# chorowski-lab/pytorch-asr

Measured on AMD Instinct MI355X. Metric: CTC train-step frames/sec, higher is better.
Workload: dtype bf16; 1 GPU; WSJ mono-char CTC (egs/wsj/yamls/ctc.yaml shapes), DeepSpeech2 conv+4xBiLSTM-320 encoder + FSTDecoder, fwd+bwd+GradientClipping(clip 480000, skip 4.8e+06 = recipe x global_batch/16)+PolyakDecay+Adam, synthetic 40-dim x 1-channel x 1000-frame fbank; batch_per_gpu=768, global_batch=768, frames=1000, classes=49, parallelism=dp1, batch_norm=per-replica statistics, optimizer_steps=139, step_boundary=device: att_speech.fused_step (clip / skip decision + Adam, no read-back)

## Files before the change

include/asr_amd.h:

```cpp
#ifndef ASR_AMD_H
#define ASR_AMD_H

#include <stdint.h>

#ifdef __cplusplus
extern "C" {
#endif

enum {
    ASR_OK = 0,
    ASR_EINVAL = 1,
    ASR_EUNSUPPORTED = 2,
    ASR_ELAUNCH = 3
};

int asr_abi_version(void);

const char *asr_strerror(int code);

int64_t asr_lattice_fwbw_workspace_bytes(int T, int B, int C, int N);

int asr_lattice_fwbw_f32(const float *lp, int T, int B, int C,
                         const int32_t *lens,
                         const int32_t *src_in, const int32_t *il_in,
// ... 169 lines not shown
int64_t asr_conv7x7c32_workspace_bytes(void);
int asr_conv7x7c32_fwd_bf16(const void *x, const float *w, int B, int H, int W, int stride_h,
                            void *y, double *chan_sums, void *workspace, int64_t workspace_bytes,
                            void *stream);
int asr_conv7x7c32_bwd_data_bf16(const void *dy, const float *w, int B, int H, int W,
                                 int stride_h, void *dx, void *workspace,
                                 int64_t workspace_bytes, void *stream);
int asr_conv7x7c32_wgrad_bf16(const void *x, const void *dy, int B, int H, int W, int stride_h,
                              float *dw, void *workspace, int64_t workspace_bytes, void *stream);

int64_t asr_conv1_7x7s2_workspace_bytes(void);
int asr_conv1_7x7s2_fwd(const float *x, const float *w, int B, int T, int F, void *y,
                        double *chan_sums, void *workspace, int64_t workspace_bytes, void *stream);
int asr_conv1_7x7s2_wgrad(const float *x, const void *dy, int B, int T, int F, float *dw,
                          void *workspace, int64_t workspace_bytes, void *stream);

int64_t asr_conv1c_7x7s2_workspace_bytes(int cin);
int asr_conv1c_7x7s2_fwd(const float *x, const float *w, int B, int T, int F, int cin, void *y,
                         double *chan_sums, void *workspace, int64_t workspace_bytes, void *stream);
int asr_conv1c_7x7s2_wgrad(const float *x, const void *dy, int B, int T, int F, int cin,
                           float *dw, void *workspace, int64_t workspace_bytes, void *stream);

int asr_tcn_attention_step_f32(const float *eproj, const float *enc, const int32_t *enc_lens,
                               const float *filt, const float *glob, const float *w_score,
                               float b_score, float temperature,
                               const float *att_prev, const int32_t *parent,
                               int T, int B, int beam, int A, int Kf, int E,
                               float *att_new, float *context, void *stream);

int asr_tcn_attention_scan_fwd_f32(const float *eproj, const float *filt, const float *glob,
// ... 123 lines not shown
```

pytorch-asr_amd/att_speech/_native.py:

```python
import ctypes
import warnings
import os

import torch

_HERE = os.path.dirname(os.path.abspath(__file__))
LIB_PATH = os.environ.get(
    'ASR_AMD_LIB', os.path.join(os.path.dirname(_HERE), 'csrc', 'libasr_amd.so'))

ASR_OK, ASR_EINVAL, ASR_EUNSUPPORTED, ASR_ELAUNCH = 0, 1, 2, 3
ABI_VERSION = 24

_lib = None
EVENT_HOOK = None
_WARNED = {}

_vp, _i, _i64, _f = ctypes.c_void_p, ctypes.c_int, ctypes.c_int64, ctypes.c_float

_SIGNATURES = {
    'asr_abi_version': (ctypes.c_int, []),
    'asr_strerror': (ctypes.c_char_p, [_i]),
    'asr_lattice_fwbw_workspace_bytes': (_i64, [_i, _i, _i, _i]),
    'asr_lattice_fwbw_f32': (_i, [_vp, _i, _i, _i, _vp, _vp, _vp, _vp, _vp, _vp,
                                  _vp, _vp, _i, _i, _i, _i, _f, _vp, _vp, _vp,
# ... 9 lines not shown
    'asr_lattice_viterbi_workspace_bytes': (_i64, [_i, _i, _i]),
    'asr_lattice_forward_f32': (_i, [_vp, _i, _i, _i, _vp, _vp, _vp, _vp, _vp,
                                     _i, _i, _i, _f, _i, _vp, _vp, _vp, _i64,
                                     _vp]),
    'asr_log_softmax_fwd_f32': (_i, [_vp, _i64, _i, _vp, _vp]),
    'asr_log_softmax_bwd_f32': (_i, [_vp, _vp, _i64, _i, _vp, _vp]),
    'asr_sub_rowmax_f32': (_i, [_vp, _i, _i, _i, _vp, _vp, _vp, _vp, _vp]),
    'asr_argmax_rows_f32': (_i, [_vp, _i64, _i, _vp, _vp]),
    'asr_conv7x7c32_workspace_bytes': (_i64, []),
    'asr_conv7x7c32_fwd_bf16': (_i, [_vp, _vp, _i, _i, _i, _i, _vp, _vp, _vp, _i64, _vp]),
    'asr_conv7x7c32_bwd_data_bf16': (_i, [_vp, _vp, _i, _i, _i, _i, _vp, _vp, _i64, _vp]),
    'asr_conv7x7c32_wgrad_bf16': (_i, [_vp, _vp, _i, _i, _i, _i, _vp, _vp, _i64, _vp]),
    'asr_conv1_7x7s2_workspace_bytes': (_i64, []),
    'asr_conv1_7x7s2_fwd': (_i, [_vp, _vp, _i, _i, _i, _vp, _vp, _vp, _i64, _vp]),
    'asr_conv1_7x7s2_wgrad': (_i, [_vp, _vp, _i, _i, _i, _vp, _vp, _i64, _vp]),
    'asr_conv1c_7x7s2_workspace_bytes': (_i64, [_i]),
    'asr_conv1c_7x7s2_fwd': (_i, [_vp, _vp, _i, _i, _i, _i, _vp, _vp, _vp, _i64, _vp]),
    'asr_conv1c_7x7s2_wgrad': (_i, [_vp, _vp, _i, _i, _i, _i, _vp, _vp, _i64, _vp]),
    'asr_log_softmax_shift_fwd_f32': (_i, [_vp, _i, _i, _i, _vp, _vp, _vp, _vp, _vp]),
    'asr_log_softmax_shift_bwd_f32': (_i, [_vp, _vp, _vp, _i64, _i, _vp, _vp]),
    'asr_sum_leading_f32': (_i, [_vp, _i, _i64, _vp, _vp]),
    'asr_adam_chunk_elems': (_i, []),
    'asr_grad_sumsq_partials_f32': (_i, [_vp, _i64, _vp, _i, _vp]),
    'asr_adam_clip_step_f32': (_i, [_vp, _i, _vp, _vp, _vp, _vp, _i, _vp, _f, _f, _f, _f, _f, _f, _f,
                                    _vp, _vp, _vp, _vp]),
    'asr_adam_clip_step_ex_f32': (_i, [_vp, _i, _vp, _vp, _vp, _vp, _i, _vp, _f, _f, _f, _f, _f, _f, _f,
                                       _vp, _vp, _vp, _vp, _vp]),
    'asr_nonfinite_flag_f32': (_i, [_vp, _i, _vp, _vp]),
    'asr_noise_chunk_elems': (_i, []),
    'asr_gaussian_noise_f32': (_i, [_vp, _i, ctypes.c_uint64, ctypes.c_uint32, ctypes.c_uint64, _i, _i, _vp]),
# ... 1120 lines not shown
    if cin == 1:
        nbytes = L.asr_conv1_7x7s2_workspace_bytes()
        ws = torch.empty(nbytes, dtype=torch.uint8, device=x.device)
        check(L.asr_conv1_7x7s2_wgrad(_p(x), _p(dy), B, T, F, _p(dw), _p(ws), nbytes, _stream()),
              'asr_conv1_7x7s2_wgrad')
    else:
        nbytes = L.asr_conv1c_7x7s2_workspace_bytes(cin)
        if nbytes < 0:
            raise NotImplementedError('conv1_wgrad: %d input channels' % cin)
        ws = torch.empty(nbytes, dtype=torch.uint8, device=x.device)
        check(L.asr_conv1c_7x7s2_wgrad(_p(x), _p(dy), B, T, F, cin, _p(dw), _p(ws), nbytes, _stream()),
              'asr_conv1c_7x7s2_wgrad')
    return dw


def split_bf16(x, hi=None, lo=None):
    x = _dev(x, torch.float32, 'x')
    if hi is None:
        hi = torch.empty(x.shape, dtype=torch.bfloat16, device=x.device)
        lo = torch.empty(x.shape, dtype=torch.bfloat16, device=x.device)
        rows, cols, ldx, ldh, ldl = 1, x.numel(), x.numel(), x.numel(), x.numel()
    else:
        if x.dim() != 2 or hi.shape != x.shape or lo.shape != x.shape or x.stride(1) != 1 \
                or hi.stride(1) != 1 or lo.stride(1) != 1 or hi.dtype != torch.bfloat16 or lo.dtype != torch.bfloat16:
            raise ValueError('split_bf16: x, hi, lo must be [rows, cols] with a dense last dimension')
        rows, cols = x.shape
        ldx, ldh, ldl = x.stride(0), hi.stride(0), lo.stride(0)
    check(lib().asr_split_bf16_f32(_p(x), rows, cols, ldx, _p(hi), ldh, _p(lo), ldl, _stream()),
          'asr_split_bf16_f32')
    return hi, lo
# ... 65 lines not shown
```

pytorch-asr_amd/att_speech/modules/encoders/deep_speech_2.py:

```python
import warnings
from collections import OrderedDict

import torch
from torch import nn

from att_speech.modules.encoders.base_encoder import BaseEncoder
from att_speech.modules.encoders.encoder_utils import (
    BatchRNN, Normalization, SequentialWithOptionalAttributes)


class DeepSpeech2(BaseEncoder):
    def __init__(self, sample_batch, conv_normalization='batch_norm',
                 conv_strides=[[2, 2], [2, 1]],
                 conv_kernel_sizes=[[41, 11], [21, 11]],
                 conv_num_features=[32, 32],
                 rnn_hidden_size=768, rnn_nb_layers=5, rnn_projection_size=0,
                 rnn_type=nn.LSTM, rnn_dropout=0.0, rnn_residual=False,
                 rnn_normalization='batch_norm', rnn_subsample=None, **kwargs):
        super(DeepSpeech2, self).__init__(**kwargs)
        import os
        self.conv_bf16 = os.environ.get('ASR_CONV_BF16', '1') != '0'
        self.fused_bn = os.environ.get('ASR_FUSED_BN', '1') != '0'
        self.native_conv = os.environ.get('ASR_NATIVE_CONV', '1') != '0'
        if isinstance(rnn_type, str):
            rnn_type = {'LSTM': nn.LSTM, 'GRU': nn.GRU}[rnn_type.split('.')[-1]]
        self.makeConv(sample_batch, conv_strides, conv_kernel_sizes,
                      conv_num_features, conv_normalization)
        features = sample_batch['features']
        features = features.permute(0, 3, 1, 2)
        with torch.no_grad():
            was_training = self.conv.training
            self.conv.eval()
            after_conv_size = self.conv.forward(features).size()
            self.conv.train(was_training)
        self.rnn_input_size = after_conv_size[1] * after_conv_size[3]
        self.makeRnn(rnn_hidden_size, rnn_nb_layers, rnn_projection_size,
                     rnn_type, rnn_dropout, rnn_residual, rnn_normalization,
                     rnn_subsample)
# ... 62 lines not shown
                                            c.dilation, c.groups)
            y = nn.functional.conv2d(
                x.to(torch.bfloat16), c.weight.to(torch.bfloat16),
                None if bias is None else bias.to(torch.bfloat16),
                c.stride, c.padding, c.dilation, c.groups)
            return y if keep_bf16 else y.float()

        def second_conv(x, with_bias=True):
            return run_conv(c2, x, with_bias)

        if fused:
            from att_speech.modules.encoders.native_bn import bn_hardtanh
            from att_speech.modules.encoders import native_conv
            c1 = conv[0]
            sums1 = sums2 = None
            if bf16 and self.native_conv and native_conv.first_supported(c1, features):
                x, sums1 = native_conv.conv1(features, c1)
            else:
                if bf16 and self.native_conv and not getattr(self, '_warned_conv1', False):
                    self._warned_conv1 = True
                    warnings.warn('DeepSpeech2: the first convolution is not a (1 or 3)->32 7x7 stride-(1,2) '
                                  'shape on gradient-free features csrc/conv.hip is built for; using '
                                  'torch / MIOpen for it')
                x = run_conv(c1, features, with_bias=False, keep_bf16=True)
            x = bn_hardtanh(x, conv[1].batch_norm, conv[2], out_bf16=bf16, conv_bias=c1.bias,
                            chan_sums=sums1)
            if bf16 and self.native_conv and native_conv.supported(c2, x):
                y2, sums2 = native_conv.conv7x7c32(x, c2)
            else:
                if bf16 and self.native_conv and not getattr(self, '_warned_conv', False):
                    self._warned_conv = True
                    warnings.warn('DeepSpeech2: the second convolution is not the 32->32 7x7 '
                                  'stride-(3,1) shape csrc/conv.hip is built for; using torch / MIOpen')
                y2 = run_conv(c2, x, with_bias=False, keep_bf16=True)
            x = bn_hardtanh(y2, conv[4].batch_norm, conv[5], time_major=True, conv_bias=c2.bias,
                            chan_sums=sums2, out_bf16=bf16 and self._rnn_takes_bf16(y2))
            return x.view(x.size(0), x.size(1), -1)
        if bf16:
            x = conv[5](conv[4](second_conv(conv[2](conv[1](conv[0](features))))))
        else:
            x = conv(features)
# ... 24 lines not shown
```

pytorch-asr_amd/att_speech/modules/encoders/native_bn.py:

```python
import torch
import torch.distributed as dist

from att_speech import _native

SYNC = {'on': False, 'group': None}


def _sync_active():
    return (SYNC['on'] and dist.is_available() and dist.is_initialized()
            and dist.get_world_size(SYNC['group']) > 1)


def _allreduce_sums(sums, n_local):
    buf = torch.cat([sums.reshape(-1), sums.new_tensor([n_local])])
    dist.all_reduce(buf, op=dist.ReduceOp.SUM, group=SYNC['group'])
    sums.copy_(buf[:-1].view_as(sums))
    return float(buf[-1])


class BNHardtanhFunction(torch.autograd.Function):
    @staticmethod
    def forward(ctx, x, gamma, beta, conv_bias, running_mean, running_var, training, momentum,
                eps, lo, hi, out_bf16, time_major, chan_sums=None, sync_counts=None):
        out, mean, invstd = _native.bn_act_fwd(
# ... 10 lines not shown
        ctx.cfg = (training, lo, hi, time_major)
        ctx.sync = training and _sync_active()
        return out

    @staticmethod
    def backward(ctx, dy):
        x, gamma, beta, mean, invstd, cb = ctx.saved_tensors
        training, lo, hi, time_major = ctx.cfg
        dx, dgamma, dbeta, dcb = _native.bn_act_bwd(
            x, gamma.detach(), beta.detach(), mean, invstd, training, lo, hi, dy,
            time_major=time_major, conv_bias=cb.detach() if ctx.has_cb else None,
            sync=_allreduce_sums if ctx.sync else None)
        return (dx, dgamma, dbeta, dcb) + (None,) * 11


def bn_hardtanh(x, bn, act, out_bf16=False, time_major=False, conv_bias=None, chan_sums=None):
    use_batch_stats = bn.training or bn.running_mean is None
    momentum = 0.0
    rm = rv = None
    if use_batch_stats and bn.training and bn.track_running_stats and bn.running_mean is not None:
        bn.num_batches_tracked.add_(1)
        momentum = bn.momentum if bn.momentum is not None else 1.0 / float(bn.num_batches_tracked)
        rm, rv = bn.running_mean, bn.running_var
    elif not use_batch_stats:
        rm, rv = bn.running_mean, bn.running_var
    if x.dtype != torch.bfloat16:
        x = x.float()
    sync_counts = None
    if use_batch_stats and bn.training and _sync_active():
        n_local = float(x.shape[0] * x.shape[2] * x.shape[3])
        if chan_sums is None:
            xd = x.double()
            chan_sums = torch.stack([xd.sum((0, 2, 3)), (xd * xd).sum((0, 2, 3))])
        else:
            chan_sums = chan_sums.clone()
        n_total = _allreduce_sums(chan_sums, n_local)
        chan_sums.mul_(n_local / n_total)
        sync_counts = (n_local, n_total)
    return BNHardtanhFunction.apply(x, bn.weight, bn.bias, conv_bias, rm, rv, use_batch_stats,
                                    momentum, bn.eps, float(act.min_val), float(act.max_val),
# ... 3 lines not shown
```

pytorch-asr_amd/att_speech/modules/encoders/native_conv.py:

```python
import torch

from att_speech import _native


def supported(conv, x):
    return (x.is_cuda and isinstance(conv, torch.nn.Conv2d) and conv.in_channels == 32
            and conv.out_channels == 32 and tuple(conv.kernel_size) == (7, 7)
            and tuple(conv.stride) == (3, 1) and tuple(conv.padding) == (0, 0)
            and tuple(conv.dilation) == (1, 1) and conv.groups == 1
            and x.dim() == 4 and x.size(2) >= 7 and 7 <= x.size(3) <= 48)


class Conv7x7C32Function(torch.autograd.Function):
    @staticmethod
    def forward(ctx, x, weight):
        x = x.to(torch.bfloat16).contiguous(memory_format=torch.channels_last)
        ctx.save_for_backward(x, weight)
        y, sums = _native.conv7x7c32_fwd(x, weight.detach(), 3, want_sums=True)
        ctx.mark_non_differentiable(sums)
        return y, sums

    @staticmethod
    def backward(ctx, dy, _dsums):
        x, weight = ctx.saved_tensors
# ... 25 lines not shown
        ctx.mark_non_differentiable(sums)
        return y, sums

    @staticmethod
    def backward(ctx, dy, _dsums):
        x, weight = ctx.saved_tensors
        return None, (_native.conv1_wgrad(x, dy) if ctx.needs_input_grad[1] else None)


def conv1(features, conv):
    if features.size(1) == 1:
        return Conv1Function.apply(features[:, 0], conv.weight)
    return Conv1Function.apply(features.permute(0, 2, 3, 1), conv.weight)


def conv7x7c32(x, conv):
    return Conv7x7C32Function.apply(x, conv.weight)
```

pytorch-asr_amd/csrc/bnact.hip:

```cpp
#include "common.h"
#include "../../include/asr_amd.h"

namespace {

using namespace asr;

struct BnParams {
    const float *x;
    int B, C, HW, Wd;
    const float *gamma, *beta;
    const float *mean, *invstd;
    const float *shift;
    float lo, hi;
};

__global__ __launch_bounds__(256) void bn_stats_kernel(const float *x, const float *shift, int C, int HW, double *sums) {
    __shared__ float red[64];
    const int c = blockIdx.x, b = blockIdx.y;
    const float *p = x + ((size_t)b * C + c) * HW;
    const float sh0 = shift ? shift[c] : 0.f;
    float s = 0.f, q = 0.f;
    for (int i = threadIdx.x; i < HW; i += 256) {
        const float v = p[i] + sh0;
        s += v;
// ... 529 lines not shown

__global__ void zero_doubles_kernel(double *p, int n) {
    const int i = blockIdx.x * blockDim.x + threadIdx.x;
    if (i < n) p[i] = 0.0;
}

inline int tm_rows(int cw) {
    if (cw <= 0) return 0;
    const int fit = 48 * 1024 / (cw * 4);
    return fit < 8 ? fit : 8;
}

inline bool bad_shape(int B, int C, int H, int W) {
    return B <= 0 || C <= 0 || H <= 0 || W <= 0 || C > 65535 || B > 65535 ||
           (int64_t)H * W > 0x7fffffff;
}

}

extern "C" int64_t asr_bn_act_workspace_bytes(int C) { return C < 0 ? -1 : (int64_t)C * 2 * 8 + 64; }

extern "C" int asr_bn_act_fwd_f32(const void *x, int x_bf16, const float *conv_bias, int B, int C, int H, int W,
                                  const float *gamma, const float *beta,
                                  float *running_mean, float *running_var,
                                  int channels_last,
                                  int training, float momentum, float eps, float lo, float hi,
                                  void *out, int out_bf16, int out_time_major,
                                  float *save_mean, float *save_invstd,
                                  const double *chan_sums,
                                  void *workspace, int64_t workspace_bytes, void *stream) {
// ... 195 lines not shown
```

pytorch-asr_amd/csrc/conv.hip:

```cpp
#include <type_traits>
#include "common.h"
#include "../../include/asr_amd.h"

namespace {

typedef __attribute__((ext_vector_type(8))) __bf16 bf16x8;
typedef __attribute__((ext_vector_type(16))) float f32x16;
typedef __attribute__((ext_vector_type(4))) unsigned int u32x4;
typedef __attribute__((ext_vector_type(4))) float f32x4;
typedef __attribute__((ext_vector_type(4))) __bf16 bf16x4;

constexpr int CH = 32;
constexpr int KS = 7;
constexpr int PIX = 80;
constexpr int KSTEPS = KS * KS * CH / 16;

typedef __attribute__((ext_vector_type(4))) int rsrc_words;
__device__ __forceinline__ rsrc_words conv_raw_rsrc(const void *base, unsigned bytes) {
    const unsigned long long a = (unsigned long long)base;
    rsrc_words r;
    r.x = __builtin_amdgcn_readfirstlane((int)(unsigned)a);
    r.y = __builtin_amdgcn_readfirstlane((int)((unsigned)(a >> 32) & 0xffffu));
    r.z = __builtin_amdgcn_readfirstlane((int)bytes);
    r.w = 0x00020000;
    return r;
// ... 671 lines not shown
        const int t = t0 - 6 + (int)row;
        bf16x8 v = {};
        if (t >= 0 && t < p.T) {
            const float2 *src = reinterpret_cast<const float2 *>(xb + (size_t)t * p.F + 2 * fo);
#pragma unroll
            for (int j = 0; j < 4; ++j) {
                const float2 f2 = src[j];
                v[2 * j] = (__bf16)f2.x;
                v[2 * j + 1] = (__bf16)f2.y;
            }
        }
        *reinterpret_cast<bf16x8 *>(wimg + (size_t)i * 16) = v;
    }
}

__global__ __launch_bounds__(256) void conv1_fwd_kernel(Conv1Params p) {
    extern __shared__ char smem[];
    const int tid = threadIdx.x, lane = tid & 63;
    const int wave = __builtin_amdgcn_readfirstlane(tid >> 6);
    const int b = blockIdx.y, t0 = blockIdx.x * C1_ROWS, Fo = p.Fo;
    const int npix = C1_ROWS * Fo, ntiles = (npix + 31) >> 5;
    char *wimg = smem;
    __bf16 *oimg = reinterpret_cast<__bf16 *>(smem + (size_t)(C1_ROWS + 8) * Fo * 16);
    bf16x8 bf[4];
#pragma unroll
    for (int s = 0; s < 4; ++s) bf[s] = reinterpret_cast<const bf16x8 *>(p.wpack)[s * 64 + lane];
    conv1_stage_windows(p, b, t0, C1_ROWS + 8, wimg, tid, 256);
    __syncthreads();
    const unsigned fmagic = (1u << 20) / (unsigned)Fo + 1u;
    for (int tile = wave; tile < ntiles; tile += 4) {
        int m = 32 * tile + (lane & 31);
        if (m >= npix) m = npix - 1;
        const unsigned r = ((unsigned)m * fmagic) >> 20, fo = (unsigned)m - r * (unsigned)Fo;
        const char *base = wimg + (size_t)((r + (unsigned)(lane >> 5)) * (unsigned)Fo + fo) * 16;
        bf16x8 a[4];
#pragma unroll
        for (int s = 0; s < 4; ++s) a[s] = *reinterpret_cast<const bf16x8 *>(base + (size_t)(2 * s * Fo) * 16);
        f32x16 acc = {};
#pragma unroll
        for (int s = 0; s < 4; ++s) acc = __builtin_amdgcn_mfma_f32_32x32x16_bf16(bf[s], a[s], acc, 0, 0, 0);
#pragma unroll
        for (int g = 0; g < 4; ++g) {
            bf16x4 o4 = {(__bf16)acc[4 * g], (__bf16)acc[4 * g + 1], (__bf16)acc[4 * g + 2], (__bf16)acc[4 * g + 3]};
            *reinterpret_cast<bf16x4 *>(reinterpret_cast<char *>(oimg) + (size_t)(32 * tile + (lane & 31)) * 64 +
                                        16 * g + 8 * (lane >> 5)) = o4;
        }
    }
    __syncthreads();
    const int rows_here = (p.To - t0) < C1_ROWS ? (p.To - t0) : C1_ROWS;
    char *yb = reinterpret_cast<char *>(p.y) + ((size_t)b * p.To + t0) * Fo * 64;
    for (int c = tid; c < rows_here * Fo * 4; c += 256)
        *reinterpret_cast<u32x4 *>(yb + (size_t)c * 16) =
            *reinterpret_cast<const u32x4 *>(reinterpret_cast<const char *>(oimg) + (size_t)c * 16);
    if (p.partial)
        chan_partial_sums(oimg, rows_here * Fo, reinterpret_cast<float *>(oimg + (size_t)ntiles * 32 * CH),
                          p.partial + ((size_t)blockIdx.y * gridDim.x + blockIdx.x) * 64);
}

constexpr int C1_WGS = 1024;
template <int DI, int WPT>
__global__ __launch_bounds__(256) void conv1_wgrad_kernel(Conv1Params p) {
    extern __shared__ char smem[];
    const int tid = threadIdx.x, lane = tid & 63;
    const int wave = __builtin_amdgcn_readfirstlane(tid >> 6);
    const int Fo = p.Fo, npix = C1_ROWS * Fo, nks = npix >> 4;
    const int nwin = (C1_ROWS + 8) * Fo;
    char *wimg = smem;
    char *dimg = smem + (size_t)nwin * 16;
    f32x16 acc[2];
#pragma unroll
    for (int t = 0; t < 2; ++t)
#pragma unroll
        for (int j = 0; j < 16; ++j) acc[t][j] = 0.f;
    const int h = lane >> 5, q = (lane & 15) >> 2, pp = lane & 3, chalf = (lane >> 4) & 1;
    const unsigned a_off = (unsigned)((8 * h + q) * PIX + (16 * chalf + 4 * pp) * 2);
    const int ktl = 2 * chalf + (pp >> 1);
    const unsigned b_lane = (unsigned)(8 * (pp & 1));
    const int chunks_per_utt = (p.To + C1_ROWS - 1) / C1_ROWS;
    const int nchunks = p.B * chunks_per_utt;
    const unsigned fmagic = (1u << 20) / (unsigned)Fo + 1u;
    u32x4 dreg[DI];
    float2 wreg[WPT][4];
    auto fetch = [&](int c) {
        const int b = c / chunks_per_utt, t0 = (c - b * chunks_per_utt) * C1_ROWS;
        const char *yb = reinterpret_cast<const char *>(p.y) + ((size_t)b * p.To + t0) * Fo * 64;
        const int rows_here = (p.To - t0) < C1_ROWS ? (p.To - t0) : C1_ROWS;
#pragma unroll
        for (int k = 0; k < DI; ++k) {
            const int i = tid + 256 * k, pix = i >> 2;
            dreg[k] = pix < rows_here * Fo ? *reinterpret_cast<const u32x4 *>(yb + (size_t)i * 16) : u32x4{0u, 0u, 0u, 0u};
        }
        const float *xb = p.x + (size_t)b * p.T * p.F;
#pragma unroll
        for (int u = 0; u < WPT; ++u) {
            const unsigned i = (unsigned)(tid + 256 * u);
            const unsigned row = (i * fmagic) >> 20, fo = i - row * (unsigned)Fo;
            const int t = t0 - 6 + (int)row;
            const bool ok = (int)i < nwin && t >= 0 && t < p.T;
            const float2 *src = reinterpret_cast<const float2 *>(xb + (size_t)(ok ? t : 0) * p.F + 2 * fo);
#pragma unroll
            for (int j = 0; j < 4; ++j) wreg[u][j] = ok ? src[j] : float2{0.f, 0.f};
        }
    };
    auto stash = [&]() {
#pragma unroll
        for (int k = 0; k < DI; ++k) {
            const int i = tid + 256 * k, pix = i >> 2, part = i & 3;
            if (pix < npix) *reinterpret_cast<u32x4 *>(dimg + pix * PIX + part * 16) = dreg[k];
        }
#pragma unroll
        for (int u = 0; u < WPT; ++u) {
            const int i = tid + 256 * u;
            bf16x8 v;
#pragma unroll
            for (int j = 0; j < 4; ++j) { v[2 * j] = (__bf16)wreg[u][j].x; v[2 * j + 1] = (__bf16)wreg[u][j].y; }
            if (i < nwin) *reinterpret_cast<bf16x8 *>(wimg + (size_t)i * 16) = v;
        }
    };
    if ((int)blockIdx.x < nchunks) fetch(blockIdx.x);
    for (int c = blockIdx.x; c < nchunks; c += gridDim.x) {
        __syncthreads();
        stash();
        __syncthreads();
        if (c + (int)gridDim.x < nchunks) fetch(c + gridDim.x);
        for (int ks = wave; ks < nks; ks += 4) {
            const bf16x8 a = tr_frag(dimg + (size_t)(16 * ks) * PIX + a_off);
            const unsigned p0 = (unsigned)(16 * ks + 8 * h + q), p1 = p0 + 4;
            const unsigned r0 = (p0 * fmagic) >> 20, f0 = p0 - r0 * (unsigned)Fo;
            const unsigned r1 = (p1 * fmagic) >> 20, f1 = p1 - r1 * (unsigned)Fo;
#pragma unroll
            for (int nt = 0; nt < 2; ++nt) {
                const int kt = 4 * nt + ktl;
                const s16x4 lo = __builtin_amdgcn_ds_read_tr16_b64_v4i16(
                    (lds_s16x4 *)(wimg + (size_t)((r0 + kt) * Fo + f0) * 16 + b_lane));
                const s16x4 hi = __builtin_amdgcn_ds_read_tr16_b64_v4i16(
                    (lds_s16x4 *)(wimg + (size_t)((r1 + kt) * Fo + f1) * 16 + b_lane));
                s16x8 v;
                v.s0 = lo.x; v.s1 = lo.y; v.s2 = lo.z; v.s3 = lo.w;
                v.s4 = hi.x; v.s5 = hi.y; v.s6 = hi.z; v.s7 = hi.w;
                acc[nt] = __builtin_amdgcn_mfma_f32_32x32x16_bf16(a, __builtin_bit_cast(bf16x8, v), acc[nt], 0, 0, 0);
            }
        }
// ... 460 lines not shown
    const int rc = conv1_shapes(B, T, F, &To, &Fo);
    if (rc != ASR_OK) return rc;
    if (!x || !dy || !dw || !workspace || workspace_bytes < asr_conv1_7x7s2_workspace_bytes())
        return ASR_EINVAL;
    hipStream_t s = (hipStream_t)stream;
    Conv1Params p;
    p.x = x; p.wpack = nullptr; p.y = (__bf16 *)const_cast<void *>(dy);
    p.partial = (float *)((char *)workspace + 4 * 64 * 8 * 2);
    p.B = B; p.T = T; p.F = F; p.To = To; p.Fo = Fo;
    size_t lds = (size_t)(C1_ROWS + 8) * Fo * 16 + (size_t)C1_ROWS * Fo * PIX;
    if (lds < 4 * 2 * 1024 * 4) lds = 4 * 2 * 1024 * 4;
    if (lds > 64 * 1024) return ASR_EUNSUPPORTED;
    const int chunks = B * ((To + C1_ROWS - 1) / C1_ROWS);
    const int nwg = chunks < C1_WGS ? chunks : C1_WGS;
    const int di = (C1_ROWS * Fo * 4 + 255) / 256, wpt = ((C1_ROWS + 8) * Fo + 255) / 256;
    void (*kern)(Conv1Params) = di <= 5 && wpt <= 2 ? conv1_wgrad_kernel<5, 2>
                              : (di <= 8 && wpt <= 3 ? conv1_wgrad_kernel<8, 3> : conv1_wgrad_kernel<16, 6>);
    hipLaunchKernelGGL(kern, dim3(nwg), dim3(256), lds, s, p);
    hipLaunchKernelGGL(conv1_wgrad_reduce_kernel, dim3(2 * 1024 / 64), dim3(1024), 0, s, p.partial, nwg, dw);
    return hipGetLastError() == hipSuccess ? ASR_OK : ASR_ELAUNCH;
}


extern "C" int64_t asr_conv1c_7x7s2_workspace_bytes(int cin) {
    if (cin != 3) return -1;
    const int64_t wg = (int64_t)C1_WGS * 2 * cin * 1024 * 4, cs = (int64_t)(1 << 17) * 64 * 4;
    return (int64_t)cin * 4 * 64 * 8 * 2 + (wg > cs ? wg : cs) + 256;
}

extern "C" int asr_conv1c_7x7s2_fwd(const float *x, const float *w, int B, int T, int F, int cin, void *y,
                                    double *chan_sums, void *workspace, int64_t workspace_bytes,
                                    void *stream) {
    int To, Fo;
// ... 64 lines not shown
```

Measured before the change: 36.01 million frames/s.

## Fuse first conv with batch-norm and hardtanh, recomputing conv output in backward

Adds a fused conv1+BN+hardtanh path for the single-channel 7x7 stride-2 first layer. The forward pass computes the conv once for channel statistics and a second time to apply BN and the activation, so the pre-BN conv output is never written to memory. The backward pass recomputes the conv inside the reduction and wgrad kernels to build the BN/activation input gradient on the fly. This removes the bf16 activation round-trip and separate BN kernels, at the cost of running the cheap single-channel conv several extra times.

```diff
diff --git a/include/asr_amd.h b/include/asr_amd.h
--- a/include/asr_amd.h
+++ b/include/asr_amd.h
@@ -207,6 +207,18 @@
                         double *chan_sums, void *workspace, int64_t workspace_bytes, void *stream);
 int asr_conv1_7x7s2_wgrad(const float *x, const void *dy, int B, int T, int F, float *dw,
                           void *workspace, int64_t workspace_bytes, void *stream);
+
+int64_t asr_conv1_bn_act_workspace_bytes(void);
+int asr_conv1_bn_act_fwd(const float *x, const float *w, const float *conv_bias, int B, int T, int F,
+                         const float *gamma, const float *beta, float *running_mean,
+                         float *running_var, float momentum, float eps, float lo, float hi,
+                         void *a1, float *save_mean, float *save_invstd, void *workspace,
+                         int64_t workspace_bytes, void *stream);
+int asr_conv1_bn_act_bwd(const float *x, const float *w, const float *conv_bias, int B, int T, int F,
+                         const float *gamma, const float *beta, const float *save_mean,
+                         const float *save_invstd, float lo, float hi, const void *da1, float *dw,
+                         float *dgamma, float *dbeta, float *dconv_bias, void *workspace,
+                         int64_t workspace_bytes, void *stream);
 
 int64_t asr_conv1c_7x7s2_workspace_bytes(int cin);
 int asr_conv1c_7x7s2_fwd(const float *x, const float *w, int B, int T, int F, int cin, void *y,
diff --git a/pytorch-asr_amd/att_speech/_native.py b/pytorch-asr_amd/att_speech/_native.py
--- a/pytorch-asr_amd/att_speech/_native.py
+++ b/pytorch-asr_amd/att_speech/_native.py
@@ -47,6 +47,11 @@
     'asr_conv1_7x7s2_workspace_bytes': (_i64, []),
     'asr_conv1_7x7s2_fwd': (_i, [_vp, _vp, _i, _i, _i, _vp, _vp, _vp, _i64, _vp]),
     'asr_conv1_7x7s2_wgrad': (_i, [_vp, _vp, _i, _i, _i, _vp, _vp, _i64, _vp]),
+    'asr_conv1_bn_act_workspace_bytes': (_i64, []),
+    'asr_conv1_bn_act_fwd': (_i, [_vp, _vp, _vp, _i, _i, _i, _vp, _vp, _vp, _vp, _f, _f, _f, _f,
+                                  _vp, _vp, _vp, _vp, _i64, _vp]),
+    'asr_conv1_bn_act_bwd': (_i, [_vp, _vp, _vp, _i, _i, _i, _vp, _vp, _vp, _vp, _f, _f, _vp, _vp,
+                                  _vp, _vp, _vp, _vp, _i64, _vp]),
     'asr_conv1c_7x7s2_workspace_bytes': (_i64, [_i]),
     'asr_conv1c_7x7s2_fwd': (_i, [_vp, _vp, _i, _i, _i, _i, _vp, _vp, _vp, _i64, _vp]),
     'asr_conv1c_7x7s2_wgrad': (_i, [_vp, _vp, _i, _i, _i, _i, _vp, _vp, _i64, _vp]),
@@ -1197,6 +1202,55 @@
     return dw
 
 
+def conv1_bn_act_fwd(x, weight, conv_bias, gamma, beta, running_mean, running_var, momentum, eps,
+                     lo, hi):
+    x = _dev(x, torch.float32, 'x')
+    weight = _dev(weight, torch.float32, 'weight')
+    if x.dim() != 3 or tuple(weight.shape) != (32, 1, 7, 7):
+        raise ValueError('conv1_bn_act_fwd: x must be [B, T, F] and weight [32, 1, 7, 7]')
+    gamma, beta = _dev(gamma, torch.float32, 'gamma'), _dev(beta, torch.float32, 'beta')
+    if conv_bias is not None:
+        conv_bias = _dev(conv_bias, torch.float32, 'conv_bias')
+    B, T, F = x.shape
+    a1 = torch.empty((B, 32, T + 6, (F - 7) // 2 + 1), dtype=torch.bfloat16, device=x.device,
+                     memory_format=torch.channels_last)
+    mean = torch.empty(32, dtype=torch.float32, device=x.device)
+    invstd = torch.empty(32, dtype=torch.float32, device=x.device)
+    L = lib()
+    nbytes = L.asr_conv1_bn_act_workspace_bytes()
+    ws = torch.empty(nbytes, dtype=torch.uint8, device=x.device)
+    check(L.asr_conv1_bn_act_fwd(_p(x), _p(weight), _p(conv_bias), B, T, F, _p(gamma), _p(beta),
+                                 _p(running_mean), _p(running_var), float(momentum), float(eps),
+                                 float(lo), float(hi), _p(a1), _p(mean), _p(invstd), _p(ws), nbytes,
+                                 _stream()), 'asr_conv1_bn_act_fwd')
+    return a1, mean, invstd
+
+
+def conv1_bn_act_bwd(x, weight, conv_bias, gamma, beta, mean, invstd, lo, hi, da1):
+    x = _dev(x, torch.float32, 'x')
+    weight = _dev(weight, torch.float32, 'weight')
+    gamma, beta = _dev(gamma, torch.float32, 'gamma'), _dev(beta, torch.float32, 'beta')
+    da1 = _nhwc_bf16(da1, 'da1')[0]
+    B, T, F = x.shape
+    if tuple(da1.shape) != (B, 32, T + 6, (F - 7) // 2 + 1):
+        raise ValueError('conv1_bn_act_bwd: da1 must be [B, 32, T + 6, (F - 7) // 2 + 1]')
+    dw = torch.empty((32, 1, 7, 7), dtype=torch.float32, device=x.device)
+    dgamma = torch.empty(32, dtype=torch.float32, device=x.device)
+    dbeta = torch.empty(32, dtype=torch.float32, device=x.device)
+    dcb = None
+    if conv_bias is not None:
+        conv_bias = _dev(conv_bias, torch.float32, 'conv_bias')
+        dcb = torch.empty(32, dtype=torch.float32, device=x.device)
+    L = lib()
+    nbytes = L.asr_conv1_bn_act_workspace_bytes()
+    ws = torch.empty(nbytes, dtype=torch.uint8, device=x.device)
+    check(L.asr_conv1_bn_act_bwd(_p(x), _p(weight), _p(conv_bias), B, T, F, _p(gamma), _p(beta),
+                                 _p(mean), _p(invstd), float(lo), float(hi), _p(da1), _p(dw),
+                                 _p(dgamma), _p(dbeta), _p(dcb), _p(ws), nbytes, _stream()),
+          'asr_conv1_bn_act_bwd')
+    return dw, dgamma, dbeta, dcb
+
+
 def split_bf16(x, hi=None, lo=None):
     x = _dev(x, torch.float32, 'x')
     if hi is None:
diff --git a/pytorch-asr_amd/att_speech/modules/encoders/deep_speech_2.py b/pytorch-asr_amd/att_speech/modules/encoders/deep_speech_2.py
--- a/pytorch-asr_amd/att_speech/modules/encoders/deep_speech_2.py
+++ b/pytorch-asr_amd/att_speech/modules/encoders/deep_speech_2.py
@@ -22,6 +22,7 @@
         self.conv_bf16 = os.environ.get('ASR_CONV_BF16', '1') != '0'
         self.fused_bn = os.environ.get('ASR_FUSED_BN', '1') != '0'
         self.native_conv = os.environ.get('ASR_NATIVE_CONV', '1') != '0'
+        self.conv1_bn = os.environ.get('ASR_CONV1_BN', '1') != '0'
         if isinstance(rnn_type, str):
             rnn_type = {'LSTM': nn.LSTM, 'GRU': nn.GRU}[rnn_type.split('.')[-1]]
         self.makeConv(sample_batch, conv_strides, conv_kernel_sizes,
@@ -114,17 +115,21 @@
             from att_speech.modules.encoders import native_conv
             c1 = conv[0]
             sums1 = sums2 = None
-            if bf16 and self.native_conv and native_conv.first_supported(c1, features):
-                x, sums1 = native_conv.conv1(features, c1)
+            if (bf16 and self.native_conv and self.conv1_bn
+                    and native_conv.conv1_bn_supported(c1, conv[1].batch_norm, features)):
+                x = native_conv.conv1_bn_hardtanh(features, c1, conv[1].batch_norm, conv[2])
             else:
-                if bf16 and self.native_conv and not getattr(self, '_warned_conv1', False):
-                    self._warned_conv1 = True
-                    warnings.warn('DeepSpeech2: the first convolution is not a (1 or 3)->32 7x7 stride-(1,2) '
-                                  'shape on gradient-free features csrc/conv.hip is built for; using '
-                                  'torch / MIOpen for it')
-                x = run_conv(c1, features, with_bias=False, keep_bf16=True)
-            x = bn_hardtanh(x, conv[1].batch_norm, conv[2], out_bf16=bf16, conv_bias=c1.bias,
-                            chan_sums=sums1)
+                if bf16 and self.native_conv and native_conv.first_supported(c1, features):
+                    x, sums1 = native_conv.conv1(features, c1)
+                else:
+                    if bf16 and self.native_conv and not getattr(self, '_warned_conv1', False):
+                        self._warned_conv1 = True
+                        warnings.warn('DeepSpeech2: the first convolution is not a (1 or 3)->32 7x7 stride-(1,2) '
+                                      'shape on gradient-free features csrc/conv.hip is built for; using '
+                                      'torch / MIOpen for it')
+                    x = run_conv(c1, features, with_bias=False, keep_bf16=True)
+                x = bn_hardtanh(x, conv[1].batch_norm, conv[2], out_bf16=bf16, conv_bias=c1.bias,
+                                chan_sums=sums1)
             if bf16 and self.native_conv and native_conv.supported(c2, x):
                 y2, sums2 = native_conv.conv7x7c32(x, c2)
             else:
diff --git a/pytorch-asr_amd/att_speech/modules/encoders/native_bn.py b/pytorch-asr_amd/att_speech/modules/encoders/native_bn.py
--- a/pytorch-asr_amd/att_speech/modules/encoders/native_bn.py
+++ b/pytorch-asr_amd/att_speech/modules/encoders/native_bn.py
@@ -48,7 +48,7 @@
         return (dx, dgamma, dbeta, dcb) + (None,) * 11
 
 
-def bn_hardtanh(x, bn, act, out_bf16=False, time_major=False, conv_bias=None, chan_sums=None):
+def running_stats_step(bn):
     use_batch_stats = bn.training or bn.running_mean is None
     momentum = 0.0
     rm = rv = None
@@ -58,6 +58,11 @@
         rm, rv = bn.running_mean, bn.running_var
     elif not use_batch_stats:
         rm, rv = bn.running_mean, bn.running_var
+    return use_batch_stats, momentum, rm, rv
+
+
+def bn_hardtanh(x, bn, act, out_bf16=False, time_major=False, conv_bias=None, chan_sums=None):
+    use_batch_stats, momentum, rm, rv = running_stats_step(bn)
     if x.dtype != torch.bfloat16:
         x = x.float()
     sync_counts = None
diff --git a/pytorch-asr_amd/att_speech/modules/encoders/native_conv.py b/pytorch-asr_amd/att_speech/modules/encoders/native_conv.py
--- a/pytorch-asr_amd/att_speech/modules/encoders/native_conv.py
+++ b/pytorch-asr_amd/att_speech/modules/encoders/native_conv.py
@@ -63,5 +63,43 @@
     return Conv1Function.apply(features.permute(0, 2, 3, 1), conv.weight)
 
 
+class Conv1BNHardtanhFunction(torch.autograd.Function):
+
+    @staticmethod
+    def forward(ctx, x, weight, gamma, beta, conv_bias, running_mean, running_var, momentum, eps,
+                lo, hi):
+        x = x.float().contiguous()
+        a1, mean, invstd = _native.conv1_bn_act_fwd(
+            x, weight.detach(), None if conv_bias is None else conv_bias.detach(), gamma.detach(),
+            beta.detach(), running_mean, running_var, momentum, eps, lo, hi)
+        ctx.has_cb = conv_bias is not None
+        ctx.save_for_backward(x, weight, gamma, beta, conv_bias if ctx.has_cb else gamma, mean, invstd)
+        ctx.cfg = (lo, hi)
+        return a1
+
+    @staticmethod
+    def backward(ctx, da1):
+        x, weight, gamma, beta, cb, mean, invstd = ctx.saved_tensors
+        dw, dgamma, dbeta, dcb = _native.conv1_bn_act_bwd(
+            x, weight.detach(), cb.detach() if ctx.has_cb else None, gamma.detach(), beta.detach(),
+            mean, invstd, ctx.cfg[0], ctx.cfg[1], da1)
+        return (None, dw, dgamma, dbeta, dcb) + (None,) * 6
+
+
+def conv1_bn_supported(conv, bn, features):
+    from att_speech.modules.encoders import native_bn
+    return (first_supported(conv, features) and conv.in_channels == 1
+            and isinstance(bn, torch.nn.BatchNorm2d) and bn.training and bn.affine
+            and not native_bn._sync_active())
+
+
+def conv1_bn_hardtanh(features, conv, bn, act):
+    from att_speech.modules.encoders.native_bn import running_stats_step
+    _, momentum, rm, rv = running_stats_step(bn)
+    return Conv1BNHardtanhFunction.apply(features[:, 0], conv.weight, bn.weight, bn.bias, conv.bias,
+                                         rm, rv, momentum, bn.eps, float(act.min_val),
+                                         float(act.max_val))
+
+
 def conv7x7c32(x, conv):
     return Conv7x7C32Function.apply(x, conv.weight)
diff --git a/pytorch-asr_amd/csrc/bn_kernels.h b/pytorch-asr_amd/csrc/bn_kernels.h
--- /dev/null
+++ b/pytorch-asr_amd/csrc/bn_kernels.h
@@ -0,0 +1,13 @@
+#pragma once
+#include <hip/hip_runtime.h>
+
+namespace asr {
+
+void bn_launch_finalize_from_sums(const double *sums, const float *shift, int C, double n, float eps,
+                                  float momentum, float *mean, float *invstd, float *running_mean,
+                                  float *running_var, hipStream_t s);
+void bn_launch_param_grads(const double *sums, int C, const float *gamma, const float *invstd,
+                           int training, float *dgamma, float *dbeta, float *dshift, hipStream_t s);
+void bn_launch_zero_doubles(double *p, int n, hipStream_t s);
+
+}
diff --git a/pytorch-asr_amd/csrc/bnact.hip b/pytorch-asr_amd/csrc/bnact.hip
--- a/pytorch-asr_amd/csrc/bnact.hip
+++ b/pytorch-asr_amd/csrc/bnact.hip
@@ -1,4 +1,5 @@
 #include "common.h"
+#include "bn_kernels.h"
 #include "../../include/asr_amd.h"
 
 namespace {
@@ -567,6 +568,27 @@
 inline bool bad_shape(int B, int C, int H, int W) {
     return B <= 0 || C <= 0 || H <= 0 || W <= 0 || C > 65535 || B > 65535 ||
            (int64_t)H * W > 0x7fffffff;
+}
+
+}
+
+namespace asr {
+
+void bn_launch_finalize_from_sums(const double *sums, const float *shift, int C, double n, float eps,
+                                  float momentum, float *mean, float *invstd, float *running_mean,
+                                  float *running_var, hipStream_t s) {
+    hipLaunchKernelGGL(bn_finalize_from_sums_kernel, dim3((C + 63) / 64), dim3(64), 0, s, sums, shift, C, n,
+                       eps, momentum, mean, invstd, running_mean, running_var);
+}
+
+void bn_launch_param_grads(const double *sums, int C, const float *gamma, const float *invstd,
+                           int training, float *dgamma, float *dbeta, float *dshift, hipStream_t s) {
+    hipLaunchKernelGGL(bn_param_grads_kernel, dim3((C + 63) / 64), dim3(64), 0, s, sums, C, gamma, invstd,
+                       training, dgamma, dbeta, dshift);
+}
+
+void bn_launch_zero_doubles(double *p, int n, hipStream_t s) {
+    hipLaunchKernelGGL(zero_doubles_kernel, dim3((n + 255) / 256), dim3(256), 0, s, p, n);
 }
 
 }
diff --git a/pytorch-asr_amd/csrc/conv.hip b/pytorch-asr_amd/csrc/conv.hip
--- a/pytorch-asr_amd/csrc/conv.hip
+++ b/pytorch-asr_amd/csrc/conv.hip
@@ -1,5 +1,6 @@
 #include <type_traits>
 #include "common.h"
+#include "bn_kernels.h"
 #include "../../include/asr_amd.h"
 
 namespace {
@@ -9,6 +10,7 @@
 typedef __attribute__((ext_vector_type(4))) unsigned int u32x4;
 typedef __attribute__((ext_vector_type(4))) float f32x4;
 typedef __attribute__((ext_vector_type(4))) __bf16 bf16x4;
+typedef __attribute__((ext_vector_type(2))) __bf16 bf16x2;
 
 constexpr int CH = 32;
 constexpr int KS = 7;
@@ -710,19 +712,18 @@
     }
 }
 
-__global__ __launch_bounds__(256) void conv1_fwd_kernel(Conv1Params p) {
-    extern __shared__ char smem[];
+template <bool STAGE>
+__device__ __forceinline__ void conv1_chunk_tile(const Conv1Params &p, int b, int t0, char *wimg, __bf16 *oimg) {
     const int tid = threadIdx.x, lane = tid & 63;
     const int wave = __builtin_amdgcn_readfirstlane(tid >> 6);
-    const int b = blockIdx.y, t0 = blockIdx.x * C1_ROWS, Fo = p.Fo;
-    const int npix = C1_ROWS * Fo, ntiles = (npix + 31) >> 5;
-    char *wimg = smem;
-    __bf16 *oimg = reinterpret_cast<__bf16 *>(smem + (size_t)(C1_ROWS + 8) * Fo * 16);
+    const int Fo = p.Fo, npix = C1_ROWS * Fo, ntiles = (npix + 31) >> 5;
     bf16x8 bf[4];
 #pragma unroll
     for (int s = 0; s < 4; ++s) bf[s] = reinterpret_cast<const bf16x8 *>(p.wpack)[s * 64 + lane];
-    conv1_stage_windows(p, b, t0, C1_ROWS + 8, wimg, tid, 256);
-    __syncthreads();
+    if (STAGE) {
+        conv1_stage_windows(p, b, t0, C1_ROWS + 8, wimg, tid, 256);
+        __syncthreads();
+    }
     const unsigned fmagic = (1u << 20) / (unsigned)Fo + 1u;
     for (int tile = wave; tile < ntiles; tile += 4) {
         int m = 32 * tile + (lane & 31);
@@ -743,6 +744,21 @@
         }
     }
     __syncthreads();
+}
+
+inline size_t conv1_tile_lds(int Fo) {
+    const int ntiles = (C1_ROWS * Fo + 31) / 32;
+    return (size_t)(C1_ROWS + 8) * Fo * 16 + (size_t)ntiles * 32 * CH * 2 + 512 * 4;
+}
+
+__global__ __launch_bounds__(256) void conv1_fwd_kernel(Conv1Params p) {
+    extern __shared__ char smem[];
+    const int tid = threadIdx.x;
+    const int b = blockIdx.y, t0 = blockIdx.x * C1_ROWS, Fo = p.Fo;
+    const int ntiles = (C1_ROWS * Fo + 31) >> 5;
+    char *wimg = smem;
+    __bf16 *oimg = reinterpret_cast<__bf16 *>(smem + (size_t)(C1_ROWS + 8) * Fo * 16);
+    conv1_chunk_tile<true>(p, b, t0, wimg, oimg);
     const int rows_here = (p.To - t0) < C1_ROWS ? (p.To - t0) : C1_ROWS;
     char *yb = reinterpret_cast<char *>(p.y) + ((size_t)b * p.To + t0) * Fo * 64;
     for (int c = tid; c < rows_here * Fo * 4; c += 256)
@@ -753,9 +769,130 @@
                           p.partial + ((size_t)blockIdx.y * gridDim.x + blockIdx.x) * 64);
 }
 
+struct Conv1BnParams {
+    const float *gamma, *beta, *mean, *invstd;
+    const float *shift;
+    float lo, hi;
+    __bf16 *out;
+    const __bf16 *da;
+    double *sums;
+    double n;
+};
+
+__global__ __launch_bounds__(256) void conv1_bn_stats_kernel(Conv1Params p) {
+    extern __shared__ char smem[];
+    const int b = blockIdx.y, t0 = blockIdx.x * C1_ROWS, Fo = p.Fo;
+    const int ntiles = (C1_ROWS * Fo + 31) >> 5;
+    char *wimg = smem;
+    __bf16 *oimg = reinterpret_cast<__bf16 *>(smem + (size_t)(C1_ROWS + 8) * Fo * 16);
+    conv1_chunk_tile<true>(p, b, t0, wimg, oimg);
+    const int rows_here = (p.To - t0) < C1_ROWS ? (p.To - t0) : C1_ROWS;
+    chan_partial_sums(oimg, rows_here * Fo, reinterpret_cast<float *>(oimg + (size_t)ntiles * 32 * CH),
+                      p.partial + ((size_t)blockIdx.y * gridDim.x + blockIdx.x) * 64);
+}
+
+__global__ __launch_bounds__(256) void conv1_bn_apply_kernel(Conv1Params p, Conv1BnParams q) {
+    extern __shared__ char smem[];
+    const int tid = threadIdx.x, c0 = 8 * (tid & 3);
+    const int b = blockIdx.y, t0 = blockIdx.x * C1_ROWS, Fo = p.Fo;
+    char *wimg = smem;
+    __bf16 *oimg = reinterpret_cast<__bf16 *>(smem + (size_t)(C1_ROWS + 8) * Fo * 16);
+    float sc[8], sh[8];
+#pragma unroll
+    for (int i = 0; i < 8; ++i) {
+        sc[i] = q.gamma[c0 + i] * q.invstd[c0 + i];
+        sh[i] = q.beta[c0 + i] - (q.mean[c0 + i] - (q.shift ? q.shift[c0 + i] : 0.f)) * sc[i];
+    }
+    conv1_chunk_tile<true>(p, b, t0, wimg, oimg);
+    const int rows_here = (p.To - t0) < C1_ROWS ? (p.To - t0) : C1_ROWS;
+    char *ob = reinterpret_cast<char *>(q.out) + ((size_t)b * p.To + t0) * Fo * 64;
+    for (int c = tid; c < rows_here * Fo * 4; c += 256) {
+        const bf16x8 v = *reinterpret_cast<const bf16x8 *>(reinterpret_cast<const char *>(oimg) + (size_t)c * 16);
+        bf16x8 o;
+#pragma unroll
+        for (int i = 0; i < 8; ++i) o[i] = (__bf16)fminf(fmaxf(fmaf((float)v[i], sc[i], sh[i]), q.lo), q.hi);
+        *reinterpret_cast<bf16x8 *>(ob + (size_t)c * 16) = o;
+    }
+}
+
+struct Conv1BnChan {
+    float m[8], is[8], g[8], be[8];
+    __device__ __forceinline__ void load(const Conv1BnParams &q, int c0) {
+#pragma unroll
+        for (int i = 0; i < 8; ++i) {
+            m[i] = q.mean[c0 + i] - (q.shift ? q.shift[c0 + i] : 0.f);
+            is[i] = q.invstd[c0 + i]; g[i] = q.gamma[c0 + i]; be[i] = q.beta[c0 + i];
+        }
+    }
+};
+
+template <int DI>
+__global__ __launch_bounds__(256) void conv1_bn_bwd_reduce_kernel(Conv1Params p, Conv1BnParams q) {
+    extern __shared__ char smem[];
+    const int tid = threadIdx.x, lane = tid & 63, c0 = 8 * (tid & 3);
+    const int wave = __builtin_amdgcn_readfirstlane(tid >> 6);
+    const int Fo = p.Fo, ntiles = (C1_ROWS * Fo + 31) >> 5;
+    char *wimg = smem;
+    __bf16 *oimg = reinterpret_cast<__bf16 *>(smem + (size_t)(C1_ROWS + 8) * Fo * 16);
+    float *red = reinterpret_cast<float *>(oimg + (size_t)ntiles * 32 * CH);
+    Conv1BnChan k;
+    k.load(q, c0);
+    float s[8], sq[8];
+#pragma unroll
+    for (int i = 0; i < 8; ++i) s[i] = sq[i] = 0.f;
+    const int chunks_per_utt = (p.To + C1_ROWS - 1) / C1_ROWS;
+    const int nchunks = p.B * chunks_per_utt;
+    for (int c = blockIdx.x; c < nchunks; c += gridDim.x) {
+        const int b = c / chunks_per_utt, t0 = (c - b * chunks_per_utt) * C1_ROWS;
+        const int rows_here = (p.To - t0) < C1_ROWS ? (p.To - t0) : C1_ROWS;
+        const int npieces = rows_here * Fo * 4;
+        const char *db = reinterpret_cast<const char *>(q.da) + ((size_t)b * p.To + t0) * Fo * 64;
+        u32x4 dreg[DI];
+#pragma unroll
+        for (int j = 0; j < DI; ++j) {
+            const int i = tid + 256 * j;
+            dreg[j] = i < npieces ? *reinterpret_cast<const u32x4 *>(db + (size_t)i * 16) : u32x4{0u, 0u, 0u, 0u};
+        }
+        __syncthreads();
+        conv1_chunk_tile<true>(p, b, t0, wimg, oimg);
+#pragma unroll
+        for (int j = 0; j < DI; ++j) {
+            const int i = tid + 256 * j;
+            if (i < npieces) {
+                const bf16x8 v = *reinterpret_cast<const bf16x8 *>(reinterpret_cast<const char *>(oimg) + (size_t)i * 16);
+                const bf16x8 dv = __builtin_bit_cast(bf16x8, dreg[j]);
+#pragma unroll
+                for (int e = 0; e < 8; ++e) {
+                    const float xh = ((float)v[e] - k.m[e]) * k.is[e];
+                    const float y = fmaf(xh, k.g[e], k.be[e]);
+                    const float d = (y > q.lo && y < q.hi) ? (float)dv[e] : 0.f;
+                    s[e] += d;
+                    sq[e] += d * xh;
+                }
+            }
+        }
+    }
+#pragma unroll
+    for (int e = 0; e < 8; ++e)
+#pragma unroll
+        for (int o = 4; o < 64; o <<= 1) {
+            s[e] += __shfl_xor(s[e], o, 64);
+            sq[e] += __shfl_xor(sq[e], o, 64);
+        }
+    __syncthreads();
+    if (lane < 4)
+#pragma unroll
+        for (int e = 0; e < 8; ++e) {
+            red[wave * 64 + 2 * (c0 + e)] = s[e];
+            red[wave * 64 + 2 * (c0 + e) + 1] = sq[e];
+        }
+    __syncthreads();
+    if (tid < 64) atomicAdd(&q.sums[tid], (double)(red[tid] + red[64 + tid] + red[128 + tid] + red[192 + tid]));
+}
+
 constexpr int C1_WGS = 1024;
-template <int DI, int WPT>
-__global__ __launch_bounds__(256) void conv1_wgrad_kernel(Conv1Params p) {
+template <int DI, int WPT, bool BN>
+__global__ __launch_bounds__(256, BN && DI <= 5 ? 3 : 1) void conv1_wgrad_kernel(Conv1Params p, Conv1BnParams q) {
     extern __shared__ char smem[];
     const int tid = threadIdx.x, lane = tid & 63;
     const int wave = __builtin_amdgcn_readfirstlane(tid >> 6);
@@ -768,8 +905,8 @@
     for (int t = 0; t < 2; ++t)
 #pragma unroll
         for (int j = 0; j < 16; ++j) acc[t][j] = 0.f;
-    const int h = lane >> 5, q = (lane & 15) >> 2, pp = lane & 3, chalf = (lane >> 4) & 1;
-    const unsigned a_off = (unsigned)((8 * h + q) * PIX + (16 * chalf + 4 * pp) * 2);
+    const int h = lane >> 5, qq = (lane & 15) >> 2, pp = lane & 3, chalf = (lane >> 4) & 1;
+    const unsigned a_off = (unsigned)((8 * h + qq) * PIX + (16 * chalf + 4 * pp) * 2);
     const int ktl = 2 * chalf + (pp >> 1);
     const unsigned b_lane = (unsigned)(8 * (pp & 1));
     const int chunks_per_utt = (p.To + C1_ROWS - 1) / C1_ROWS;
@@ -777,6 +914,17 @@
     const unsigned fmagic = (1u << 20) / (unsigned)Fo + 1u;
     u32x4 dreg[DI];
     float2 wreg[WPT][4];
+    float *ctab = reinterpret_cast<float *>(dimg + (npix * PIX > ((npix + 31) >> 5) * 32 * 64 ? npix * PIX : ((npix + 31) >> 5) * 32 * 64));
+    if (BN && tid < CH) {
+        const float is = q.invstd[tid], g = q.gamma[tid];
+        ctab[0 * CH + tid] = q.mean[tid] - (q.shift ? q.shift[tid] : 0.f);
+        ctab[1 * CH + tid] = is;
+        ctab[2 * CH + tid] = g;
+        ctab[3 * CH + tid] = q.beta[tid];
+        ctab[4 * CH + tid] = (float)(q.sums[2 * tid] / q.n);
+        ctab[5 * CH + tid] = (float)(q.sums[2 * tid + 1] / q.n);
+        ctab[6 * CH + tid] = g * is;
+    }
     auto fetch = [&](int c) {
         const int b = c / chunks_per_utt, t0 = (c - b * chunks_per_utt) * C1_ROWS;
         const char *yb = reinterpret_cast<const char *>(p.y) + ((size_t)b * p.To + t0) * Fo * 64;
@@ -798,12 +946,47 @@
             for (int j = 0; j < 4; ++j) wreg[u][j] = ok ? src[j] : float2{0.f, 0.f};
         }
     };
-    auto stash = [&]() {
+    auto stash_dy = [&]() {
 #pragma unroll
         for (int k = 0; k < DI; ++k) {
             const int i = tid + 256 * k, pix = i >> 2, part = i & 3;
             if (pix < npix) *reinterpret_cast<u32x4 *>(dimg + pix * PIX + part * 16) = dreg[k];
         }
+    };
+    auto make_dy = [&](int c) {
+        const int t0 = (c % chunks_per_utt) * C1_ROWS;
+        const int rows_here = (p.To - t0) < C1_ROWS ? (p.To - t0) : C1_ROWS;
+        u32x4 yreg[DI];
+#pragma unroll
+        for (int j = 0; j < DI; ++j) {
+            const int i = tid + 256 * j;
+            yreg[j] = (i >> 2) < npix ? *reinterpret_cast<const u32x4 *>(dimg + (size_t)i * 16) : u32x4{0u, 0u, 0u, 0u};
+        }
+        __syncthreads();
+#pragma unroll
+        for (int hq = 0; hq < 4; ++hq) {
+            float2 cst[7];
+#pragma unroll
+            for (int a = 0; a < 7; ++a) cst[a] = *reinterpret_cast<const float2 *>(ctab + a * CH + 8 * (tid & 3) + 2 * hq);
+#pragma unroll
+            for (int j = 0; j < DI; ++j) {
+                const bf16x2 v = __builtin_bit_cast(bf16x2, yreg[j][hq]), dv = __builtin_bit_cast(bf16x2, dreg[j][hq]);
+                bf16x2 o;
+#pragma unroll
+                for (int e = 0; e < 2; ++e) {
+                    const float m = e ? cst[0].y : cst[0].x, is = e ? cst[1].y : cst[1].x, g = e ? cst[2].y : cst[2].x;
+                    const float be = e ? cst[3].y : cst[3].x, k1 = e ? cst[4].y : cst[4].x, k2 = e ? cst[5].y : cst[5].x;
+                    const float gi = e ? cst[6].y : cst[6].x;
+                    const float xh = ((float)v[e] - m) * is;
+                    const float y = fmaf(xh, g, be);
+                    const float d = (y > q.lo && y < q.hi) ? (float)dv[e] : 0.f;
+                    o[e] = (__bf16)(gi * (d - k1 - xh * k2));
+                }
+                dreg[j][hq] = ((tid + 256 * j) >> 2) < rows_here * Fo ? __builtin_bit_cast(unsigned, o) : 0u;
+            }
+        }
+    };
+    auto stash_windows = [&]() {
 #pragma unroll
         for (int u = 0; u < WPT; ++u) {
             const int i = tid + 256 * u;
@@ -816,12 +999,19 @@
     if ((int)blockIdx.x < nchunks) fetch(blockIdx.x);
     for (int c = blockIdx.x; c < nchunks; c += gridDim.x) {
         __syncthreads();
-        stash();
+        if (!BN) stash_dy();
+        stash_windows();
+        if (BN) {
+            __syncthreads();
+            conv1_chunk_tile<false>(p, 0, 0, wimg, reinterpret_cast<__bf16 *>(dimg));
+            make_dy(c);
+            stash_dy();
+        }
         __syncthreads();
         if (c + (int)gridDim.x < nchunks) fetch(c + gridDim.x);
         for (int ks = wave; ks < nks; ks += 4) {
             const bf16x8 a = tr_frag(dimg + (size_t)(16 * ks) * PIX + a_off);
-            const unsigned p0 = (unsigned)(16 * ks + 8 * h + q), p1 = p0 + 4;
+            const unsigned p0 = (unsigned)(16 * ks + 8 * h + qq), p1 = p0 + 4;
             const unsigned r0 = (p0 * fmagic) >> 20, f0 = p0 - r0 * (unsigned)Fo;
             const unsigned r1 = (p1 * fmagic) >> 20, f1 = p1 - r1 * (unsigned)Fo;
 #pragma unroll
@@ -1312,9 +1502,106 @@
     const int chunks = B * ((To + C1_ROWS - 1) / C1_ROWS);
     const int nwg = chunks < C1_WGS ? chunks : C1_WGS;
     const int di = (C1_ROWS * Fo * 4 + 255) / 256, wpt = ((C1_ROWS + 8) * Fo + 255) / 256;
-    void (*kern)(Conv1Params) = di <= 5 && wpt <= 2 ? conv1_wgrad_kernel<5, 2>
-                              : (di <= 8 && wpt <= 3 ? conv1_wgrad_kernel<8, 3> : conv1_wgrad_kernel<16, 6>);
-    hipLaunchKernelGGL(kern, dim3(nwg), dim3(256), lds, s, p);
+    void (*kern)(Conv1Params, Conv1BnParams) =
+        di <= 5 && wpt <= 2 ? conv1_wgrad_kernel<5, 2, false>
+                            : (di <= 8 && wpt <= 3 ? conv1_wgrad_kernel<8, 3, false> : conv1_wgrad_kernel<16, 6, false>);
+    hipLaunchKernelGGL(kern, dim3(nwg), dim3(256), lds, s, p, Conv1BnParams{});
+    hipLaunchKernelGGL(conv1_wgrad_reduce_kernel, dim3(2 * 1024 / 64), dim3(1024), 0, s, p.partial, nwg, dw);
+    return hipGetLastError() == hipSuccess ? ASR_OK : ASR_ELAUNCH;
+}
+
+
+extern "C" int64_t asr_conv1_bn_act_workspace_bytes(void) {
+    return asr_conv1_7x7s2_workspace_bytes() + 64 * 8 + 256;
+}
+
+static double *conv1_bn_sums(void *workspace) {
+    return (double *)((char *)workspace + asr_conv1_7x7s2_workspace_bytes());
+}
+
+extern "C" int asr_conv1_bn_act_fwd(const float *x, const float *w, const float *conv_bias, int B, int T,
+                                    int F, const float *gamma, const float *beta, float *running_mean,
+                                    float *running_var, float momentum, float eps, float lo, float hi,
+                                    void *a1, float *save_mean, float *save_invstd, void *workspace,
+                                    int64_t workspace_bytes, void *stream) {
+    int To, Fo;
+    const int rc = conv1_shapes(B, T, F, &To, &Fo);
+    if (rc != ASR_OK) return rc;
+    if (!x || !w || !gamma || !beta || !a1 || !save_mean || !save_invstd || !workspace ||
+        workspace_bytes < asr_conv1_bn_act_workspace_bytes() || (!running_mean) != (!running_var))
+        return ASR_EINVAL;
+    const dim3 grid((To + C1_ROWS - 1) / C1_ROWS, B);
+    if (B > 65535 || (int64_t)grid.x * grid.y * 64 * 4 > asr_conv1_7x7s2_workspace_bytes() - 4 * 64 * 8 * 2 - 256)
+        return ASR_EUNSUPPORTED;
+    const size_t lds = conv1_tile_lds(Fo);
+    if (lds > 64 * 1024) return ASR_EUNSUPPORTED;
+    hipStream_t s = (hipStream_t)stream;
+    __bf16 *wpack = (__bf16 *)workspace;
+    hipLaunchKernelGGL(conv1_pack_kernel, dim3(8), dim3(256), 0, s, w, wpack);
+    Conv1Params p;
+    p.x = x; p.wpack = wpack; p.y = nullptr;
+    p.partial = (float *)((char *)workspace + 4 * 64 * 8 * 2);
+    p.B = B; p.T = T; p.F = F; p.To = To; p.Fo = Fo;
+    double *sums = conv1_bn_sums(workspace);
+    hipLaunchKernelGGL(conv1_bn_stats_kernel, grid, dim3(256), lds, s, p);
+    hipLaunchKernelGGL(zero_chan_sums_kernel, dim3(1), dim3(64), 0, s, sums);
+    hipLaunchKernelGGL(chan_sums_reduce_kernel, dim3(64), dim3(1024), 0, s, p.partial, (int)(grid.x * grid.y), sums);
+    asr::bn_launch_finalize_from_sums(sums, conv_bias, CH, (double)B * (To * Fo), eps, momentum, save_mean,
+                                      save_invstd, running_mean, running_var, s);
+    Conv1BnParams q{};
+    q.gamma = gamma; q.beta = beta; q.mean = save_mean; q.invstd = save_invstd; q.shift = conv_bias;
+    q.lo = lo; q.hi = hi; q.out = (__bf16 *)a1;
+    hipLaunchKernelGGL(conv1_bn_apply_kernel, grid, dim3(256), lds, s, p, q);
+    return hipGetLastError() == hipSuccess ? ASR_OK : ASR_ELAUNCH;
+}
+
+extern "C" int asr_conv1_bn_act_bwd(const float *x, const float *w, const float *conv_bias, int B, int T,
+                                    int F, const float *gamma, const float *beta, const float *save_mean,
+                                    const float *save_invstd, float lo, float hi, const void *da1,
+                                    float *dw, float *dgamma, float *dbeta, float *dconv_bias,
+                                    void *workspace, int64_t workspace_bytes, void *stream) {
+    int To, Fo;
+    const int rc = conv1_shapes(B, T, F, &To, &Fo);
+    if (rc != ASR_OK) return rc;
+    if (!x || !w || !gamma || !beta || !save_mean || !save_invstd || !da1 || !dw || !dgamma || !dbeta ||
+        !workspace || workspace_bytes < asr_conv1_bn_act_workspace_bytes())
+        return ASR_EINVAL;
+    const size_t lds_red = conv1_tile_lds(Fo);
+    const int npix = C1_ROWS * Fo, ntiles = (npix + 31) / 32;
+    const size_t dimg = (size_t)npix * PIX, oimg = (size_t)ntiles * 32 * CH * 2;
+    size_t lds = (size_t)(C1_ROWS + 8) * Fo * 16 + (dimg > oimg ? dimg : oimg) + 7 * CH * 4;
+    if (lds < 4 * 2 * 1024 * 4) lds = 4 * 2 * 1024 * 4;
+    if (lds > 64 * 1024 || lds_red > 64 * 1024) return ASR_EUNSUPPORTED;
+    hipStream_t s = (hipStream_t)stream;
+    __bf16 *wpack = (__bf16 *)workspace;
+    hipLaunchKernelGGL(conv1_pack_kernel, dim3(8), dim3(256), 0, s, w, wpack);
+    Conv1Params p;
+    p.x = x; p.wpack = wpack; p.y = (__bf16 *)const_cast<void *>(da1);
+    p.partial = (float *)((char *)workspace + 4 * 64 * 8 * 2);
+    p.B = B; p.T = T; p.F = F; p.To = To; p.Fo = Fo;
+    Conv1BnParams q{};
+    q.gamma = gamma; q.beta = beta; q.mean = save_mean; q.invstd = save_invstd; q.shift = conv_bias;
+    q.lo = lo; q.hi = hi; q.da = (const __bf16 *)da1; q.sums = conv1_bn_sums(workspace);
+    q.n = (double)B * (To * Fo);
+    const int chunks = B * ((To + C1_ROWS - 1) / C1_ROWS);
+    const int di = (C1_ROWS * Fo * 4 + 255) / 256, wpt = ((C1_ROWS + 8) * Fo + 255) / 256;
+    asr::bn_launch_zero_doubles(q.sums, 2 * CH, s);
+    int cus = conv_cu_count();
+    if (cus <= 0) cus = 256;
+    const int per_cu = di <= 5 ? 3 : (di <= 8 ? 2 : 1);
+    {
+        const int nwg = chunks < per_cu * cus ? chunks : per_cu * cus;
+        void (*kern)(Conv1Params, Conv1BnParams) =
+            di <= 5 ? conv1_bn_bwd_reduce_kernel<5> : (di <= 8 ? conv1_bn_bwd_reduce_kernel<8> : conv1_bn_bwd_reduce_kernel<16>);
+        hipLaunchKernelGGL(kern, dim3(nwg), dim3(256), lds_red, s, p, q);
+    }
+    asr::bn_launch_param_grads(q.sums, CH, gamma, save_invstd, 1, dgamma, dbeta, dconv_bias, s);
+    int nwg = chunks < per_cu * cus ? chunks : per_cu * cus;
+    if (nwg > C1_WGS) nwg = C1_WGS;
+    void (*kern)(Conv1Params, Conv1BnParams) =
+        di <= 5 && wpt <= 2 ? conv1_wgrad_kernel<5, 2, true>
+                            : (di <= 8 && wpt <= 3 ? conv1_wgrad_kernel<8, 3, true> : conv1_wgrad_kernel<16, 6, true>);
+    hipLaunchKernelGGL(kern, dim3(nwg), dim3(256), lds, s, p, q);
     hipLaunchKernelGGL(conv1_wgrad_reduce_kernel, dim3(2 * 1024 / 64), dim3(1024), 0, s, p.partial, nwg, dw);
     return hipGetLastError() == hipSuccess ? ASR_OK : ASR_ELAUNCH;
 }
```

Measured after the change: 36.45 million frames/s, median of 6. 1.01x the previous value.
